# beer-asr/beer

Hardware: AMD Instinct MI355X
Metric: frames/sec per VB iteration (E+M) (higher is better)
Workload: dtype f32

## Files before the change

### beer_amd/csrc/estep_bf16.hip

```cpp

#include <cstdlib>
#include <type_traits>
#include <utility>

#include "estep_mfma.h"
#include "estep_tiles.h"

namespace beer_mfma {

namespace {

typedef __bf16 bf8 __attribute__((ext_vector_type(8)));
typedef unsigned int u4 __attribute__((ext_vector_type(4)));
typedef float f32x2 __attribute__((ext_vector_type(2)));

template <int V> using ic = std::integral_constant<int, V>;
template <int... I, typename F>
__device__ __forceinline__ void static_for_impl(std::integer_sequence<int, I...>, F&& f) {
    (f(ic<I>{}), ...);
}
template <int N, typename F>
__device__ __forceinline__ void static_for(F&& f) {
    static_for_impl(std::make_integer_sequence<int, N>{}, static_cast<F&&>(f));
}

constexpr int NP = kPackedPieces;
constexpr int kProdA[6] = {0, 0, 1, 0, 1, 2};
constexpr int kProdB[6] = {0, 1, 0, 2, 1, 0};

__device__ __forceinline__ bf8 as_bf8(const u4& w) { return __builtin_bit_cast(bf8, w); }
__device__ __forceinline__ f32x4 mfma_bf16(const u4& a, const u4& b, const f32x4& c) {
    return __builtin_amdgcn_mfma_f32_16x16x32_bf16(as_bf8(a), as_bf8(b), c, 0, 0, 0);
}
template <bool FIRST>
__device__ __forceinline__ void mfma_bf16_pinned(f32x4& acc, const u4& a, const u4& b) {
    if (FIRST)
        asm volatile("s_nop 1\n\tv_mfma_f32_16x16x32_bf16 %0, %1, %2, %0" : "+a"(acc) : "v"(a), "v"(b));
    else
        asm volatile("v_mfma_f32_16x16x32_bf16 %0, %1, %2, %0" : "+a"(acc) : "v"(a), "v"(b));
}
__device__ __forceinline__ void mfma_drain() {
    asm volatile("s_nop 15\n\ts_nop 15" ::: "memory");
    __builtin_amdgcn_sched_barrier(0);
}

__host__ __device__ inline size_t frame_image_tile_u4(int nk_used, int nqt) {
    return (size_t)(nk_used * NP * 2 + nqt * NP) * 64;
}
__host__ __device__ constexpr int img_nqt(int nk_used) { return nk_used <= 3 ? 5 : 6; }
constexpr int kImgMaxNK = 4;
__host__ __device__ inline int stat_slab(int j) { return j + j / 7; }
__host__ __device__ inline int nk16_of(int cov, int D) {
    return ((nslabx_of(cov, D) + 7) / 8 + 1) / 2 * 2;
}
__host__ __device__ inline int ld16_of(int D) {
    const int ld = 4 * d4_of(D) + 8;
    return (ld / 4) % 2 ? ld : ld + 4;
}
constexpr float kConstEps = 5.9604644775390625e-8f;
constexpr int kBlockU4 = NP * 64;

__device__ inline double entry_value(int cov, int D, int K, int k, int slab, int e,
                                     const float* __restrict__ row, bool* is_const) {
    const int D4 = d4_of(D), Dp = 4 * D4, nslab = nslabx_of(cov, D);
    *is_const = false;
    if (slab >= nslab) return 0.0;
    if (band_layout(cov, D)) {
        const int nb = band_nslab(D);
        if (slab == nslab - 1) {
            *is_const = true;
            return 0.0;
        }
        if (k >= K) return 0.0;
        if (slab >= nb) {
            const int b = 4 * (slab - nb) + e;
            return b < D ? (double)row[b] : 0.0;
        }
        int a, b;
        if (!band_pair(D, slab, e, &a, &b)) return 0.0;
        return b == a ? -0.5 * (double)row[D + a * D + a]
                      : -0.5 * ((double)row[D + a * D + b] + (double)row[D + b * D + a]);
    }
    const int t = slab_entry(cov, D, slab);
    const int a = t & 0xff, b = ((t >> 8) & 0xff) + e, sq = t >> 16;
    if (a == Dp && b - e == Dp) {
        *is_const = true;
        return 0.0;
    }
    if (k >= K) return 0.0;
    if (sq) return b < D ? -0.5 * (double)row[cov == BEER_ISO ? D : D + b] : 0.0;
    if (a < D) {
        if (b >= D || b < a) return 0.0;
        return b == a ? -0.5 * (double)row[D + a * D + a]
                      : -0.5 * ((double)row[D + a * D + b] + (double)row[D + b * D + a]);
    }
    return b < D ? (double)row[b] : 0.0;
}

__global__ __launch_bounds__(256) void const_max_kernel(int cov, int D, int K,
                                                        const float* __restrict__ E,
                                                        const float* __restrict__ logw,
                                                        float* __restrict__ c0) {
    __shared__ double red[8];
    const int Q = stats_dim(cov, D);
    double m = -1.0e300;
    for (int k = threadIdx.x; k < K; k += blockDim.x) {
        const double v = const_total(cov, D, E + (size_t)k * Q, logw ? (double)logw[k] : 0.0);
        if (v == v && v > m && v < 1.0e300) m = v;
    }
    m = block_max(m, red);
    if (threadIdx.x == 0) c0[0] = m > -1.0e300 ? (float)m : 0.f;
}

__global__ __launch_bounds__(256) void packx_kernel(int cov, int D, int K, int NT,
                                                    const float* __restrict__ E,
                                                    const float* __restrict__ logw,
                                                    unsigned short* __restrict__ P,
                                                    int* __restrict__ tab, int G, int Gp,
                                                    const float* __restrict__ c0, int lane_major) {
    extern __shared__ __attribute__((aligned(16))) char pack_lds[];
    const int nk = nk16_of(cov, D), nent = nk * 32;
    const int slot = blockIdx.x;
    const int k = slot % Gp < G ? (slot / Gp) * G + slot % Gp : K;
    const int chunk = slot / (NT * 16), kk = slot % (NT * 16);
    const int c = lane_major ? kk % NT : 4 * (kk / 64) + (kk % 4);
    const int i = lane_major ? kk / NT : (kk % 64) / 4;
    if (slot == 0)
        for (int s = threadIdx.x; s < (nk + 1) * 8; s += blockDim.x) tab[s] = slabx_entry(cov, D, s);
    const int Qs = stats_dim(cov, D);
    float* rowl = reinterpret_cast<float*>(pack_lds);
    if (k < K)
        for (int q = threadIdx.x; q < Qs; q += blockDim.x) rowl[q] = E[(size_t)k * Qs + q];
    __syncthreads();
    unsigned short* base = P + ((size_t)chunk * nk * NT) * (NP * 512);
    auto put = [&](int q, float v) {
        const int s = q / 32, g = (q % 32) / 8, j = q % 8;
        unsigned short* dst = base + ((size_t)s * NT + c) * (NP * 512) + (g * 16 + i) * 8 + j;
        unsigned short p[3];
        split3_scalar(v, p);
        dst[0] = p[0];
        dst[512] = p[1];
        dst[1024] = p[2];
    };
    const int nslab = nslabx_of(cov, D);
    for (int q = threadIdx.x; q < nent; q += blockDim.x) {
        bool is_const;
        const double v = entry_value(cov, D, K, k, q / 4, q % 4, rowl, &is_const);
        if (!is_const) {
            put(q, (float)v);
        } else if (q % 4 == 0) {
            const bool last = q / 4 == nslab - 1;
            const double want = k < K ? const_share(cov, D, q / 4, rowl, logw ? (double)logw[k] : 0.0) -
                                            (last ? (double)c0[0] : 0.0)
                                      : (last ? kPadLogit : 0.0);
            const float hi = (float)want;
            const double rem = (want - (double)hi) * (1.0 / (double)kConstEps);
            put(q, hi);
            put(q + 1, (rem == rem && fabs(rem) < 1.0e30) ? (float)rem : 0.f);
            put(q + 2, 0.f);
            put(q + 3, 0.f);
        }
    }
}

inline int xcd_chunk_group(int ny, size_t chunk_bytes) {
    int cg = (int)((size_t)(2 << 20) / (chunk_bytes ? chunk_bytes : 1));
    return cg < 1 ? 1 : (cg > ny ? ny : cg);
}
inline unsigned xcd_grid(int64_t nx, int ny, int cg) {
    return (unsigned)((nx + 7) / 8 * 8 * cg * ((ny + cg - 1) / cg));
}
__device__ inline bool xcd_block(int64_t nx, int ny, int cg, int64_t& bx, int& by) {
    const unsigned per_group = (unsigned)((nx + 7) / 8 * 8 * cg);
    const unsigned grp = blockIdx.x / per_group, rem = blockIdx.x - grp * per_group;
    const unsigned xcd = rem & 7, slot = rem >> 3;
    by = (int)(grp * cg + slot % (unsigned)cg);
    bx = (int64_t)(slot / (unsigned)cg) * 8 + xcd;
    return bx < nx && by < ny;
}

template <int FW>
__device__ __forceinline__ void stage_rows(const float* __restrict__ X, int64_t fb,
                                           int64_t nframes, int D, int LD, int lane,
                                           float* __restrict__ xw) {
    const int Dp = 4 * d4_of(D);
    if ((D & 3) == 0) {
        constexpr int LPR = 64 / FW, NPC = kMaxDimX / 4 / LPR;
        const int C4 = D >> 2, r = lane & (FW - 1), h = lane / FW;
        const int64_t f = fb + r;
        const bool valid = f < nframes;
        const f32x4* src = reinterpret_cast<const f32x4*>(X) + (valid ? f : nframes - 1) * C4;
        f32x4 xv[NPC];
#pragma unroll
        for (int it = 0; it < NPC; ++it) {
            const int pc = h + LPR * it;
            xv[it] = src[pc < C4 ? pc : C4 - 1];
        }
#pragma unroll
        for (int it = 0; it < NPC; ++it) {
            const int pc = h + LPR * it;
            if (pc < C4)
                *reinterpret_cast<f32x4*>(xw + r * LD + 4 * pc) =
                    valid ? xv[it] : f32x4{0.f, 0.f, 0.f, 0.f};
        }
        for (int idx = lane; idx < FW * ((LD - D) / 4); idx += 64) {
            const int rr = idx / ((LD - D) / 4), hh = idx - rr * ((LD - D) / 4);
            *reinterpret_cast<f32x4*>(xw + rr * LD + D + 4 * hh) =
                f32x4{hh == 0 ? 1.f : 0.f, hh == 0 ? kConstEps : 0.f, 0.f, 0.f};
        }
    } else {
        for (int idx = lane; idx < FW * LD; idx += 64) {
            const int r = idx / LD, c = idx - r * LD;
            const int64_t f = fb + r;
            float v = 0.f;
            if (c < D) { if (f < nframes) v = X[f * D + c]; }
            else if (c == Dp) v = 1.f;
            else if (c == Dp + 1) v = kConstEps;
            xw[idx] = v;
        }
    }
}

template <int NT, int MT, int GQ, bool PACKED, bool SQ, bool LNO, bool IMG = false, bool BL = false>
__global__ __launch_bounds__(kThreads, 2) void llhx_kernel(
    int64_t nframes, int D, int K, int S, int G, int gl, int jw, int nk,
    const float* __restrict__ X, const u4* __restrict__ Pall, const int* __restrict__ tab,
    float* __restrict__ resps, float* __restrict__ log_norm, double* __restrict__ llh_sum,
    float* __restrict__ xt_out, int xt_floats, int nku, int cg, const float* __restrict__ c0,
    const u4* __restrict__ img = nullptr) {
    static_assert(MT * NT <= 32, "128 accumulators: two waves per SIMD (launch bounds)");
    static_assert(!IMG || (MT == 2 && !PACKED && LNO), "the image holds 32-frame tiles");
    static_assert(!BL || (NT == 16 && MT == 2 && !IMG), "half k-steps of 8 tiles, hipcc-scheduled form");
    extern __shared__ __attribute__((aligned(16))) char smem[];
    const int LD = ld16_of(D);
    const int Dp = 4 * d4_of(D);
    const int tid = threadIdx.x, lane = tid & 63;
    const int wave = __builtin_amdgcn_readfirstlane(tid >> 6);
    const int i = lane & 15, g = lane >> 4;
    constexpr int FW = 16 * MT, NW = kThreads / 64;
    float* xw = reinterpret_cast<float*>(smem) + wave * (FW * LD);
    int* tabs = reinterpret_cast<int*>(reinterpret_cast<float*>(smem) + NW * FW * LD);
    constexpr int kHalfBytes = 8 * kBlockU4 * 16;
    char* ring = smem + (((size_t)NW * FW * LD * sizeof(float) + (size_t)(nk + 1) * 8 * sizeof(int)
                          + 1023) & ~(size_t)1023);
    int64_t bx = blockIdx.x;
    int by = 0;
    {
        const int nch = (K + 16 * NT - 1) / (16 * NT);
        constexpr int FBK = FW * NW;
        if (nch > 1 && !xcd_block((nframes + FBK - 1) / FBK, nch, cg, bx, by)) return;
    }
    const int64_t fb = (bx * NW + wave) * FW;
    for (int idx = tid; idx < (nk + 1) * 8; idx += kThreads) tabs[idx] = tab[idx];
    if (!IMG) stage_rows<FW>(X, fb, nframes, D, LD, lane, xw);
    __syncthreads();
    if (IMG && fb >= nframes) return;
    {
        static_assert(64 % FW == 0, "whole waves per 64-frame tile");
        if (xt_out && by == 0 && fb < (nframes + 63) / 64 * 64) {
            float* img = xt_out + (fb / 64) * (size_t)xt_floats;
            const int c0 = (int)(fb % 64);
            const int ncol4 = FW / 4 + (c0 + FW == 64 ? 1 : 0);
            for (int e4 = lane; e4 < (D + 2) * ncol4; e4 += 64) {
                const int row = e4 / ncol4, c = 4 * (e4 - row * ncol4);
                f32x4 v = {0.f, 0.f, 0.f, 0.f};
                if (row < D) {
#pragma unroll
                    for (int j = 0; j < 4; ++j) v[j] = c + j < FW ? xw[(c + j) * LD + row] : 0.f;
                } else if (row == D) {
                    v = f32x4{1.f, 1.f, 1.f, 1.f};
                }
                __builtin_nontemporal_store(v, reinterpret_cast<f32x4*>(img + row * 68 + c0 + c));
            }
        }
    }

    f32x4 acc[MT][NT];
#pragma unroll
    for (int m = 0; m < MT; ++m)
#pragma unroll
        for (int c = 0; c < NT; ++c) acc[m][c] = f32x4{0, 0, 0, 0};

    const float* xrow[MT];
#pragma unroll
    for (int m = 0; m < MT; ++m) xrow[m] = xw + (m * 16 + i) * LD;

    const int kbase = by * (16 * NT);
    const u4* Pl = Pall + (size_t)by * nk * NT * kBlockU4 + lane;
    const int* tl = tabs + 2 * g;

    struct AFrag { u4 w[NP][MT]; };
    auto make_half = [&](int s, int m, int h, AFrag& f) {
        const int t = tl[8 * s + h];
        f32x4 p;
        if constexpr (SQ) {
            const int a = t & 0xff, j = (t >> 8) & 0xff;
            const bool sq = (t >> 16) != 0;
            const f32x4 bb = *reinterpret_cast<const f32x4*>(xrow[m] + j);
            const float xx = xrow[m][a];
#pragma unroll
            for (int e = 0; e < 4; ++e) p[e] = bb[e] * (sq ? bb[e] : xx);
        } else {
            const f32x4 bb = *reinterpret_cast<const f32x4*>(xrow[m] + (t & 0xff));
#pragma unroll
            for (int e = 0; e < 4; ++e) p[e] = bb[e] * xrow[m][band_col(t, e, Dp)];
        }
#pragma unroll
        for (int e = 0; e < 2; ++e) {
            unsigned w3[3];
            split3(p[2 * e], p[2 * e + 1], w3);
#pragma unroll
            for (int q = 0; q < NP; ++q) f.w[q][m][2 * h + e] = w3[q];
        }
    };
    constexpr int BT = 2, NBATCH = NT / BT;
    static_assert(NT % BT == 0 && NBATCH % 2 == 0, "B batches alternate between two buffers");
    struct BFrag { u4 p[BT][NP]; };
    auto load_b = [&](int64_t blk, BFrag& b) {
#pragma unroll
        for (int c = 0; c < BT; ++c)
#pragma unroll
            for (int q = 0; q < NP; ++q) {
                if constexpr (BL) {
                    const int bb = (int)(blk + c);
                    b.p[c][q] = *reinterpret_cast<const u4*>(
                        ring + ((bb >> 3) & 1) * kHalfBytes + (bb & 7) * (kBlockU4 * 16) + q * 1024 +
                        lane * 16);
                } else {
                    b.p[c][q] = Pl[(size_t)(blk + c) * kBlockU4 + 64 * q];
                }
            }
    };
    typedef __attribute__((address_space(3))) void* lds_ptr;
    const char* bsrc = reinterpret_cast<const char*>(Pall + (size_t)by * nk * NT * kBlockU4) +
                       wave * 1024 + lane * 16;
    auto stage_half = [&](int hs) {
        const char* src = bsrc + (size_t)hs * kHalfBytes;
        char* dst = ring + (hs & 1) * kHalfBytes + wave * 1024;
#pragma unroll
        for (int n = 0; n < kHalfBytes / 1024 / NW; ++n)
            __builtin_amdgcn_global_load_lds(reinterpret_cast<const u4*>(src + n * (NW * 1024)),
                                             (lds_ptr)(dst + n * (NW * 1024)), 16, 0, 0);
    };
    auto publish = [&]() {
        asm volatile("s_waitcnt vmcnt(0) lgkmcnt(0)" ::: "memory");
        __builtin_amdgcn_s_barrier();
    };
    auto batch = [&](int s, int bi, const AFrag& cur, AFrag& nxt, const BFrag& b, BFrag& bn) {
        if constexpr (BL) {
            if (bi == NBATCH / 2 - 1 || bi == NBATCH - 1) {
                publish();
                const int hs = 2 * (s + 1) + (bi == NBATCH - 1 ? 1 : 0);
                if (hs < 2 * nku) stage_half(hs);
            }
        }
        load_b((int64_t)s * NT + (bi + 1) * BT, bn);
        if constexpr (!IMG) {
#pragma unroll
            for (int hh = bi * MT * 2 / NBATCH; hh < (bi + 1) * MT * 2 / NBATCH; ++hh)
                make_half(s + 1, hh % MT, hh / MT, nxt);
        }
#pragma unroll
        for (int pr = 0; pr < 6; ++pr)
#pragma unroll
            for (int c = 0; c < BT; ++c)
#pragma unroll
                for (int m = 0; m < MT; ++m)
                    acc[m][bi * BT + c] = mfma_bf16(cur.w[kProdA[pr]][m], b.p[c][kProdB[pr]],
                                                    acc[m][bi * BT + c]);
        if constexpr (BL)
            __builtin_amdgcn_sched_group_barrier(0x100, NP * BT, 0);
        else
            __builtin_amdgcn_sched_group_barrier(0x020, NP * BT, 0);
        if constexpr (!IMG)
            __builtin_amdgcn_sched_group_barrier(0x100, 2 * ((MT * 2 + NBATCH - 1) / NBATCH), 0);
        __builtin_amdgcn_sched_group_barrier(0x008, 6 * MT * BT, 0);
    };
    const u4* ti = nullptr;
    if constexpr (IMG)
        ti = img + (fb / FW) * (int64_t)frame_image_tile_u4(nku, img_nqt(nku)) + lane;
    auto load_a = [&](int s, AFrag& f) {
#pragma unroll
        for (int q = 0; q < NP; ++q)
#pragma unroll
            for (int m = 0; m < MT; ++m) f.w[q][m] = ti[((s * NP + q) * MT + m) * 64];
    };
    auto kstep = [&](int s, const AFrag& cur, AFrag& nxt, BFrag& b0, BFrag& b1) {
        if constexpr (IMG) {
            if (s + 1 < nku) load_a(s + 1, nxt);
        }
#pragma unroll
        for (int bi = 0; bi < NBATCH; bi += 2) {
            batch(s, bi, cur, nxt, b0, b1);
            batch(s, bi + 1, cur, nxt, b1, b0);
        }
    };
    AFrag f0, f1;
    BFrag b0, b1;
    if constexpr (IMG) {
        load_a(0, f0);
    } else {
#pragma unroll
        for (int hh = 0; hh < MT * 2; ++hh) make_half(0, hh % MT, hh / MT, f0);
    }
    if constexpr (BL) {
        stage_half(0);
        if (nku > 0) stage_half(1);
        publish();
    }
    load_b(0, b0);
    for (int s = 0; s < nku; s += 2) {
        kstep(s, f0, f1, b0, b1);
        if (s + 1 < nku) kstep(s + 1, f1, f0, b0, b1);
    }
    if constexpr (LNO) {
        if constexpr (NT == 16 && GQ == 1) {
            if (gl == 0) {
                if (G == 4)
                    lognorm_epilogue_lane_major<NT, MT, 4>(acc, fb, nframes, kbase, S, i, g, lane, log_norm, llh_sum, c0[0]);
                else if (G == 8)
                    lognorm_epilogue_lane_major<NT, MT, 8>(acc, fb, nframes, kbase, S, i, g, lane, log_norm, llh_sum, c0[0]);
                else
                    lognorm_epilogue_lane_major<NT, MT, 16>(acc, fb, nframes, kbase, S, i, g, lane, log_norm, llh_sum, c0[0]);
                return;
            }
        }
#define BEER_LN(GL_) lognorm_epilogue<NT, MT, GQ, GL_>(acc, fb, nframes, kbase, S, G, i, g, lane, \
                                                       log_norm, llh_sum, c0[0])
        switch (gl) {
            case 1: BEER_LN(1); break;
            case 2: BEER_LN(2); break;
            case 4: BEER_LN(4); break;
            case 8: BEER_LN(8); break;
            default: BEER_LN(16); break;
        }
#undef BEER_LN
    } else {
        softmax_epilogue<float, NT, MT, GQ, PACKED, LNO>(acc, fb, nframes, kbase, K, S, G, gl, jw,
                                                         i, g, lane, resps, log_norm, llh_sum,
                                                         c0[0]);
    }
}

inline bool k1_lds_fits(int D, int nk) {
    size_t lds = (size_t)32 * (kThreads / 64) * ld16_of(D) * sizeof(float) + (size_t)(nk + 1) * 8 * sizeof(int);
    lds = ((lds + 1023) & ~(size_t)1023) + 2 * (size_t)(8 * kBlockU4 * 16);
    return 2 * lds <= (size_t)beer::kMaxDynLds;
}

thread_local int g_cov_of_launch = BEER_FULL;

template <int NT, int MT, int GQ, bool PACKED = false, bool SQ = true, bool LNO = false,
          bool IMG = false, bool BL = false>
int launch_llhx(int64_t nframes, int D, int K, int S, int G, int gl, int jw, int nchunks, int nk,
                const float* X, const void* P, const int* tab, const float* c0, float* resps,
                float* log_norm, double* llh_sum, hipStream_t s, float* xt_out = nullptr,
                int xt_floats = 0, const void* img = nullptr) {
    const int LD = ld16_of(D);
    const int nku = (nslabx_of(SQ ? g_cov_of_launch : BEER_FULL, D) + 7) / 8;
    constexpr int FB = 16 * MT * (kThreads / 64);
    size_t lds = (size_t)FB * LD * sizeof(float) + (size_t)(nk + 1) * 8 * sizeof(int);
    if (BL) lds = ((lds + 1023) & ~(size_t)1023) + 2 * (size_t)(8 * kBlockU4 * 16);
    const int64_t blocks = (nframes + FB - 1) / FB;
    if (nchunks != (K + 16 * NT - 1) / (16 * NT)) return BEER_EINVAL;
    const int cg = xcd_chunk_group(nchunks, (size_t)nku * NT * kBlockU4 * 16);
    (void)hipFuncSetAttribute(
        reinterpret_cast<const void*>(llhx_kernel<NT, MT, GQ, PACKED, SQ, LNO, IMG, BL>),
        hipFuncAttributeMaxDynamicSharedMemorySize, beer::kMaxDynLds);
    hipLaunchKernelGGL((llhx_kernel<NT, MT, GQ, PACKED, SQ, LNO, IMG, BL>),
                       dim3(nchunks > 1 ? xcd_grid(blocks, nchunks, cg) : (unsigned)blocks),
                       dim3(kThreads), lds, s, nframes, D, K, S, G, gl, jw, nk, X,
                       reinterpret_cast<const u4*>(P), tab, resps, log_norm, llh_sum, xt_out,
                       xt_floats, nku, cg, c0, reinterpret_cast<const u4*>(img));
    BEER_LAUNCH_CHECK();
    return BEER_OK;
}

constexpr int kAxFT = 64;
constexpr int kAxXS = kAxFT + 4;
constexpr int kPiece = 4096;
constexpr int kAxMC = 8, kAxWaves = 4;

inline int xt_rows(int D) { return D + 2; }
inline int xt_pieces(int D) { return (xt_rows(D) * kAxXS * 4 + kPiece - 1) / kPiece; }

__global__ __launch_bounds__(256) void xt_image_kernel(int64_t nframes, int D, int NX,
                                                       const float* __restrict__ X,
                                                       float* __restrict__ Xt) {
    constexpr int LD = kMaxDimX + 1;
    __shared__ float tile[kAxFT * LD];
    const int64_t tau = blockIdx.x, t0 = tau * kAxFT;
    const int rows = (int)(nframes - t0 < kAxFT ? nframes - t0 : kAxFT);
    for (int e = threadIdx.x; e < rows * D; e += 256) {
        const int f = e / D, d = e - f * D;
        tile[f * LD + d] = X[t0 * D + e];
    }
    __syncthreads();
    float* out = Xt + tau * ((size_t)NX * (kPiece / 4));
    for (int e = threadIdx.x; e < NX * (kPiece / 4); e += 256) {
        const int row = e / kAxXS, col = e - row * kAxXS;
        float v = 0.f;
        if (row < D) v = col < rows ? tile[col * LD + row] : 0.f;
        else if (row == D) v = 1.f;
        __builtin_nontemporal_store(v, out + e);
    }
}

template <bool SR, int NQ>
__global__ __launch_bounds__(64 * kAxWaves, 1) void accx_kernel(
    int64_t nframes, int D, int K, int nslab, int NX, const float* __restrict__ Xt,
    const unsigned* __restrict__ Rimg, const int* __restrict__ tab,
    int64_t frames_per_block, double* __restrict__ Sp, int gx, int gy, int gz,
    const float* __restrict__ Gt, int lgG, int sx, int band) {
    constexpr int MC = kAxMC, WAVES = kAxWaves, NB = 2;
    static_assert(16 * MC == kPackedComps && kAxFT == kPackedFrames, "the packed image is this kernel's LDS tile");
    constexpr int plane = kPackedPlaneWords * 4;
    const int r_off = NX * kPiece, buf_bytes = r_off + NP * plane;
    const int xstride = sx ? 0 : buf_bytes;
    const int rstride = sx ? NP * plane : buf_bytes;
    const int g_base = sx ? r_off + NB * NP * plane : NB * buf_bytes;
    extern __shared__ __attribute__((aligned(16))) char smem[];
    const int tid = threadIdx.x, lane = tid & 63;
    const int wave = __builtin_amdgcn_readfirstlane(tid >> 6);
    const int i = lane & 15, g = lane >> 4;
    const int D4 = d4_of(D), Dp = 4 * D4, nq = nslab * 4;
    const int id = blockIdx.x, xcd = id & 7, slot0 = id >> 3;
    const int bx = slot0 % gx;
    const int yz = (slot0 / gx) * 8 + xcd;
    if (yz >= gy * gz) return;
    const int by = yz % gy, bz = yz / gy;
    const int tile0 = (bx * WAVES + wave) * NQ;
    const int kc0 = by * (16 * MC);
    const int64_t tb = (int64_t)bz * frames_per_block;
    const int64_t te = tb + frames_per_block < nframes ? tb + frames_per_block : nframes;
    const int ntiles = (int)((te - tb + kAxFT - 1) / kAxFT);
    const int64_t tau0 = tb / kAxFT;
    const int nblk = (K + 16 * MC - 1) / (16 * MC);
    const int gbytes = SR ? ((16 * MC) >> lgG) * kAxFT * 4 : 0;
    const int gkb = (gbytes + 1023) >> 10;

    auto factors = [&](int uu, int& a, int& b) {
        const int col = 16 * (tile0 + uu) + i, slab = col >> 2;
        a = b = Dp + 2;
        if (slab < nslab) {
            const int t = tab[slab];
            if (band) {
                a = (t & 0xff) + (col & 3);
                b = band_col(t, col & 3, Dp);
            } else {
                b = ((t >> 8) & 0xff) + (col & 3);
                a = (t >> 16) ? b : (t & 0xff);
            }
        }
    };
    int xa_off[NQ], xb_off[NQ];
#pragma unroll
    for (int uu = 0; uu < NQ; ++uu) {
        int a, b;
        factors(uu, a, b);
        xa_off[uu] = ((a < D ? a : (a == Dp ? D : D + 1)) * kAxXS + 8 * g) * 4;
        xb_off[uu] = ((b < D ? b : (b == Dp ? D : D + 1)) * kAxXS + 8 * g) * 4;
    }
    int a_off[kAxFT / 32];
#pragma unroll
    for (int ks = 0; ks < kAxFT / 32; ++ks)
        a_off[ks] = r_off + (i * kPackedFrames + (((4 * ks + g) ^ (i & 7)) << 3)) * 2;

    f32x4 acc[MC][NQ];
#pragma unroll
    for (int c = 0; c < MC; ++c)
#pragma unroll
        for (int uu = 0; uu < NQ; ++uu) acc[c][uu] = f32x4{0, 0, 0, 0};

    static_assert((kPiece / 1024) % WAVES == 0 && (NP * plane / 1024) % WAVES == 0,
                  "regions are whole rounds of the waves");
    const char* xsrc = reinterpret_cast<const char*>(Xt) + wave * 1024 + lane * 16;
    const char* rsrc = reinterpret_cast<const char*>(Rimg) + wave * 1024 + lane * 16;
    const char* gsrc = SR ? reinterpret_cast<const char*>(Gt) + wave * 1024 + lane * 16 : nullptr;
    typedef __attribute__((address_space(3))) void* lds_ptr;
    auto stage_x = [&](int tile, int buf) {
        const char* xs = xsrc + (tau0 + tile) * (size_t)(NX * kPiece);
        char* dst = smem + buf * xstride + wave * 1024;
#pragma unroll 1
        for (int n = 0; n < NX * (kPiece / 1024) / WAVES; ++n)
            __builtin_amdgcn_global_load_lds(reinterpret_cast<const u4*>(xs + n * (WAVES * 1024)),
                                             (lds_ptr)(dst + n * (WAVES * 1024)), 16, 0, 0);
    };
    auto stage_r = [&](int tile, int buf) {
        const int64_t tau = tau0 + tile;
        const char* rs = rsrc + (tau * nblk + by) * (size_t)(NP * plane);
        char* dst = smem + r_off + buf * rstride + wave * 1024;
#pragma unroll
        for (int n = 0; n < NP * plane / 1024 / WAVES; ++n)
            __builtin_amdgcn_global_load_lds(reinterpret_cast<const u4*>(rs + n * (WAVES * 1024)),
                                             (lds_ptr)(dst + n * (WAVES * 1024)), 16, 0, 0);
        if (SR && wave < gkb)
            __builtin_amdgcn_global_load_lds(
                reinterpret_cast<const u4*>(gsrc + (tau * nblk + by) * (size_t)gbytes),
                (lds_ptr)(smem + g_base + buf * 4096 + wave * 1024), 16, 0, 0);
    };
    auto stage = [&](int tile, int buf) {
        if (!sx) stage_x(tile, buf);
        stage_r(tile, buf);
    };
    auto fold = [&](int buf) {
#pragma unroll 1
        for (int n = 0; n < 16 * MC * 8 / (64 * WAVES); ++n) {
            const int p = tid + 64 * WAVES * n, c = p >> 3, pos = p & 7, ch = pos ^ (c & 7);
            char* ph = smem + buf * rstride + r_off + c * (kPackedFrames * 2) + pos * 16;
            const u4 w0 = *reinterpret_cast<const u4*>(ph);
            const u4 w1 = *reinterpret_cast<const u4*>(ph + plane);
            const u4 w2 = *reinterpret_cast<const u4*>(ph + 2 * plane);
            const float* gm = reinterpret_cast<const float*>(smem + g_base + buf * 4096) +
                              ((c >> lgG) * kAxFT + 8 * ch);
            const f32x4 g0 = *reinterpret_cast<const f32x4*>(gm);
            const f32x4 g1 = *reinterpret_cast<const f32x4*>(gm + 4);
            u4 o0, o1, o2;
#pragma unroll
            for (int wd = 0; wd < 4; ++wd) {
                const float lo = (__builtin_bit_cast(float, w1[wd] << 16) +
                                  __builtin_bit_cast(float, w2[wd] << 16)) +
                                 __builtin_bit_cast(float, w0[wd] << 16);
                const float hi = (__builtin_bit_cast(float, w1[wd] & 0xffff0000u) +
                                  __builtin_bit_cast(float, w2[wd] & 0xffff0000u)) +
                                 __builtin_bit_cast(float, w0[wd] & 0xffff0000u);
                const float ga = wd < 2 ? g0[2 * wd] : g1[2 * wd - 4];
                const float gb = wd < 2 ? g0[2 * wd + 1] : g1[2 * wd - 3];
                unsigned w3[3];
                split3(lo * ga, hi * gb, w3);
                o0[wd] = w3[0]; o1[wd] = w3[1]; o2[wd] = w3[2];
            }
            *reinterpret_cast<u4*>(ph) = o0;
            *reinterpret_cast<u4*>(ph + plane) = o1;
            *reinterpret_cast<u4*>(ph + 2 * plane) = o2;
        }
    };
    if (ntiles > 0) {
        stage_x(0, 0);
        stage_r(0, 0);
    }
    __syncthreads();
    if (SR && ntiles > 0) {
        fold(0);
        __syncthreads();
    }
    const bool active = tile0 * 16 < nq;
    u4 af[MC][NP], bf[2][NP];
    constexpr int kPA[6] = {0, 0, 0, 1, 1, 2}, kPB[6] = {0, 1, 2, 0, 1, 0};
    auto a_ptr = [&](int b, int ks, int c) {
        return smem + a_off[ks] + (b * rstride + c * 16 * kPackedFrames * 2);
    };
    auto load_a = [&](int b, int ks) {
#pragma unroll
        for (int q = 0; q < NP; ++q)
#pragma unroll
            for (int c = 0; c < MC; ++c)
                af[c][q] = *reinterpret_cast<const u4*>(a_ptr(b, ks, c) + q * plane);
    };
    auto gen_b = [&](int b, int ks, int uu, u4 (&out)[NP]) {
        const char* pa = smem + xa_off[uu] + (b * xstride + 128 * ks);
        const char* pb = smem + xb_off[uu] + (b * xstride + 128 * ks);
        const f32x4 xa0 = *reinterpret_cast<const f32x4*>(pa);
        const f32x4 xa1 = *reinterpret_cast<const f32x4*>(pa + 16);
        const f32x4 xb0 = *reinterpret_cast<const f32x4*>(pb);
        const f32x4 xb1 = *reinterpret_cast<const f32x4*>(pb + 16);
        const f32x4 p0 = xa0 * xb0, p1 = xa1 * xb1;
#pragma unroll
        for (int e = 0; e < 4; ++e) {
            unsigned w3[3];
            split3(e < 2 ? p0[2 * e] : p1[2 * e - 4], e < 2 ? p0[2 * e + 1] : p1[2 * e - 3], w3);
#pragma unroll
            for (int q = 0; q < NP; ++q) out[q][e] = w3[q];
        }
    };
    if (active && ntiles > 0) gen_b(0, 0, 0, bf[0]);
    auto iteration = [&](int tile, int buf) __attribute__((always_inline)) {
        const int next = buf ^ 1;
        if (tile + 1 < ntiles) stage(tile + 1, next);
        const bool fold_next = SR && tile + 1 < ntiles;
        if (active) {
#pragma unroll
            for (int ks = 0; ks < 2; ++ks) {
                load_a(buf, ks);
#pragma unroll
                for (int uu = 0; uu < NQ; ++uu) {
                    const int cur = (ks * NQ + uu) & 1;
                    const bool build = uu + 1 < NQ || ks == 0;
                    const int nks = uu + 1 < NQ ? ks : 1, nuu = uu + 1 < NQ ? uu + 1 : 0;
                    const char* pa = smem + xa_off[nuu] + (buf * xstride + 128 * nks);
                    const char* pb = smem + xb_off[nuu] + (buf * xstride + 128 * nks);
                    f32x4 xa[2], xb[2];
                    float pp[8];
                    Split3Steps st[4];
#pragma unroll
                    for (int n = 0; n < 6 * MC; ++n) {
                        const int pr = n / MC, c = n % MC;
                        mfma_bf16_pinned<false>(acc[c][uu], af[c][kPA[pr]], bf[cur][kPB[pr]]);
                        if (!build) continue;
                        if (n == 1) xa[0] = *reinterpret_cast<const f32x4*>(pa);
                        else if (n == 2) xa[1] = *reinterpret_cast<const f32x4*>(pa + 16);
                        else if (n == 3) xb[0] = *reinterpret_cast<const f32x4*>(pb);
                        else if (n == 4) xb[1] = *reinterpret_cast<const f32x4*>(pb + 16);
                        else if (n >= 12 && n < 20) {
                            const int e = n - 12;
                            asm volatile("v_mul_f32 %0, %1, %2" : "=v"(pp[e])
                                         : "v"(xa[e >> 2][e & 3]), "v"(xb[e >> 2][e & 3]));
                        } else if (n >= 20) {
                            constexpr int NCH = 2;
                            const int m = n - 20, grp = m / (7 * NCH), mm = m % (7 * NCH);
                            const int e = NCH * grp + mm % NCH;
                            split3_step(mm / NCH, pp[2 * e], pp[2 * e + 1], st[e]);
                        }
                    }
                    if (build) {
#pragma unroll
                        for (int e = 0; e < 4; ++e) {
                            bf[cur ^ 1][0][e] = st[e].w0;
                            bf[cur ^ 1][1][e] = st[e].w1;
                            bf[cur ^ 1][2][e] = st[e].w2;
                        }
                    }
                }
            }
        }
        __syncthreads();
        if (sx && tile + 1 < ntiles) {
            stage_x(tile + 1, 0);
            __syncthreads();
        }
        if (SR) {
            if (fold_next) fold(next);
            __syncthreads();
        }
        if (active && tile + 1 < ntiles) gen_b(next, 0, 0, bf[0]);
    };
    for (int tile = 0; tile < ntiles; tile += NB) {
        iteration(tile, 0);
        if (tile + 1 < ntiles) iteration(tile + 1, 1);
    }
    mfma_drain();
#pragma unroll
    for (int uu = 0; uu < NQ; ++uu) {
        const int q = (tile0 + uu) * 16 + i;
        if (q >= nq) continue;
#pragma unroll
        for (int c = 0; c < MC; ++c)
#pragma unroll
// ... 1392 lines not shown
```

Baseline: 247.0 million.

## Hand-interleave A-fragment generation and B loads with pinned MFMAs in BL path

For the band-layout (BL) kernel variant, each batch becomes a hand-scheduled stream. Pinned inline-asm MFMAs are interleaved with LDS loads of the next B fragments, address computation, raw X loads and split3 steps for the next A fragment. The table words are pre-packed into 6-bit column indices so addresses come from bitfield extracts rather than band_col evaluation. This hides the fragment-building latency behind MFMA issue, but it relies on manual hazard handling (s_nop, drain) and is restricted to leading dimensions of 64 or less and non-SQ configurations.

```diff
diff --git a/beer_amd/csrc/estep_bf16.hip b/beer_amd/csrc/estep_bf16.hip
--- a/beer_amd/csrc/estep_bf16.hip
+++ b/beer_amd/csrc/estep_bf16.hip
@@ -38,6 +38,9 @@
         asm volatile("s_nop 1\n\tv_mfma_f32_16x16x32_bf16 %0, %1, %2, %0" : "+a"(acc) : "v"(a), "v"(b));
     else
         asm volatile("v_mfma_f32_16x16x32_bf16 %0, %1, %2, %0" : "+a"(acc) : "v"(a), "v"(b));
+}
+__device__ __forceinline__ void mfma_bf16_pinned_v(f32x4& acc, const u4& a, const u4& b) {
+    asm volatile("v_mfma_f32_16x16x32_bf16 %0, %1, %2, %0" : "+v"(acc) : "v"(a), "v"(b));
 }
 __device__ __forceinline__ void mfma_drain() {
     asm volatile("s_nop 15\n\ts_nop 15" ::: "memory");
@@ -221,6 +224,13 @@
     }
 }
 
+__device__ __forceinline__ int k1_slab_word(int t, int Dp) {
+    int w = t & 0xff;
+#pragma unroll
+    for (int e = 0; e < 4; ++e) w |= band_col(t, e, Dp) << (6 + 6 * e);
+    return w;
+}
+
 template <int NT, int MT, int GQ, bool PACKED, bool SQ, bool LNO, bool IMG = false, bool BL = false>
 __global__ __launch_bounds__(kThreads, 2) void llhx_kernel(
     int64_t nframes, int D, int K, int S, int G, int gl, int jw, int nk,
@@ -230,7 +240,7 @@
     const u4* __restrict__ img = nullptr) {
     static_assert(MT * NT <= 32, "128 accumulators: two waves per SIMD (launch bounds)");
     static_assert(!IMG || (MT == 2 && !PACKED && LNO), "the image holds 32-frame tiles");
-    static_assert(!BL || (NT == 16 && MT == 2 && !IMG), "half k-steps of 8 tiles, hipcc-scheduled form");
+    static_assert(!BL || (NT == 16 && MT == 2 && !IMG && !SQ), "half k-steps of 8 tiles, band slabs");
     extern __shared__ __attribute__((aligned(16))) char smem[];
     const int LD = ld16_of(D);
     const int Dp = 4 * d4_of(D);
@@ -251,7 +261,8 @@
         if (nch > 1 && !xcd_block((nframes + FBK - 1) / FBK, nch, cg, bx, by)) return;
     }
     const int64_t fb = (bx * NW + wave) * FW;
-    for (int idx = tid; idx < (nk + 1) * 8; idx += kThreads) tabs[idx] = tab[idx];
+    for (int idx = tid; idx < (nk + 1) * 8; idx += kThreads)
+        tabs[idx] = BL ? k1_slab_word(tab[idx], Dp) : tab[idx];
     if (!IMG) stage_rows<FW>(X, fb, nframes, D, LD, lane, xw);
     __syncthreads();
     if (IMG && fb >= nframes) return;
@@ -301,9 +312,10 @@
 #pragma unroll
             for (int e = 0; e < 4; ++e) p[e] = bb[e] * (sq ? bb[e] : xx);
         } else {
-            const f32x4 bb = *reinterpret_cast<const f32x4*>(xrow[m] + (t & 0xff));
-#pragma unroll
-            for (int e = 0; e < 4; ++e) p[e] = bb[e] * xrow[m][band_col(t, e, Dp)];
+            const f32x4 bb = *reinterpret_cast<const f32x4*>(xrow[m] + (t & (BL ? 0x3f : 0xff)));
+#pragma unroll
+            for (int e = 0; e < 4; ++e)
+                p[e] = bb[e] * xrow[m][BL ? (t >> (6 + 6 * e)) & 0x3f : band_col(t, e, Dp)];
         }
 #pragma unroll
         for (int e = 0; e < 2; ++e) {
@@ -346,13 +358,80 @@
         asm volatile("s_waitcnt vmcnt(0) lgkmcnt(0)" ::: "memory");
         __builtin_amdgcn_s_barrier();
     };
+    static_assert(!BL || 4 * MT == NBATCH, "one unit of fragment arithmetic per batch");
+    struct ARaw { f32x4 bb; float xc[4]; };
+    typedef __attribute__((address_space(3))) const float* lds_cf;
+    typedef __attribute__((address_space(3))) const f32x4* lds_cf4;
+    ARaw raw[2];
+    int th[2];
+    unsigned ad[5], rowb[MT];
+#pragma unroll
+    for (int m = 0; m < MT; ++m) rowb[m] = (unsigned)(size_t)(lds_cf)xrow[m];
+    auto addr_step = [&](int k, int m, int h) {
+#define BEER_AD(K_, LO_)                                                                     \
+    case K_:                                                                                 \
+        asm volatile("v_bfe_u32 %0, %1, " #LO_ ", 6\n\tv_lshl_add_u32 %0, %0, 2, %2"         \
+                     : "=&v"(ad[K_]) : "v"(th[h]), "v"(rowb[m]));                            \
+        break;
+        switch (k) {
+            BEER_AD(0, 0) BEER_AD(1, 6) BEER_AD(2, 12) BEER_AD(3, 18) BEER_AD(4, 24)
+            default: break;
+        }
+#undef BEER_AD
+    };
+    auto load_raw = [&](int k, ARaw& r) {
+        if (k == 0) r.bb = *(lds_cf4)ad[0];
+        else r.xc[k - 1] = *(lds_cf)ad[k];
+    };
+    auto batch_stream = [&](int s, int bi, const AFrag& cur, AFrag& nxt, const BFrag& b, BFrag& bn) {
+        if (bi == NBATCH / 2 - 1 || bi == NBATCH - 1) {
+            publish();
+            const int hs = 2 * (s + 1) + (bi == NBATCH - 1 ? 1 : 0);
+            if (hs < 2 * nku) stage_half(hs);
+        }
+        const int bb0 = s * NT + (bi + 1) * BT;
+        const int hu = bi / 2, mu = hu % MT, wu = 2 * (hu / MT) + bi % 2, eu = bi % 2;
+        const ARaw& ru = raw[hu & 1];
+        const int hl = (bi / 2 + 1) % (MT * 2);
+        float pp[2];
+        Split3Steps st;
+#pragma unroll
+        for (int n = 0; n < 6 * MT * BT; ++n) {
+            const int pr = n / (MT * BT), c = n / MT % BT, m = n % MT, k = n / 2;
+            mfma_bf16_pinned_v(acc[m][bi * BT + c], cur.w[kProdA[pr]][m], b.p[c][kProdB[pr]]);
+            if (n % 2 == 0) {
+                const int kb = bi % 2 ? k - 5 : k - 1;
+                if (kb >= 0 && kb < NP * BT) {
+                    const int blk = bb0 + kb % BT;
+                    bn.p[kb % BT][kb / BT] = *reinterpret_cast<const u4*>(
+                        ring + ((blk >> 3) & 1) * kHalfBytes + (blk & 7) * (kBlockU4 * 16) +
+                        (kb / BT) * 1024 + lane * 16);
+                } else if (bi % 2) {
+                    if (k < 5) load_raw(k, raw[hl & 1]);
+                } else if (k >= 7) {
+                    addr_step(k - 7, hl % MT, hl / MT);
+                } else if (bi == NBATCH / 2 - 2) {
+                    th[1] = tl[8 * (s + 1) + 1];
+                } else if (bi == NBATCH - 2) {
+                    th[0] = tl[8 * min(s + 2, nk)];
+                }
+            } else if (k == 0) {
+                asm volatile("v_mul_f32 %0, %2, %3\n\tv_mul_f32 %1, %4, %5"
+                             : "=&v"(pp[0]), "=&v"(pp[1])
+                             : "v"(ru.bb[2 * eu]), "v"(ru.xc[2 * eu]), "v"(ru.bb[2 * eu + 1]),
+                               "v"(ru.xc[2 * eu + 1]));
+            } else if (k < 8) {
+                split3_step(k - 1, pp[0], pp[1], st);
+            }
+        }
+        nxt.w[0][mu][wu] = st.w0;
+        nxt.w[1][mu][wu] = st.w1;
+        nxt.w[2][mu][wu] = st.w2;
+    };
     auto batch = [&](int s, int bi, const AFrag& cur, AFrag& nxt, const BFrag& b, BFrag& bn) {
         if constexpr (BL) {
-            if (bi == NBATCH / 2 - 1 || bi == NBATCH - 1) {
-                publish();
-                const int hs = 2 * (s + 1) + (bi == NBATCH - 1 ? 1 : 0);
-                if (hs < 2 * nku) stage_half(hs);
-            }
+            batch_stream(s, bi, cur, nxt, b, bn);
+            return;
         }
         load_b((int64_t)s * NT + (bi + 1) * BT, bn);
         if constexpr (!IMG) {
@@ -368,10 +447,7 @@
                 for (int m = 0; m < MT; ++m)
                     acc[m][bi * BT + c] = mfma_bf16(cur.w[kProdA[pr]][m], b.p[c][kProdB[pr]],
                                                     acc[m][bi * BT + c]);
-        if constexpr (BL)
-            __builtin_amdgcn_sched_group_barrier(0x100, NP * BT, 0);
-        else
-            __builtin_amdgcn_sched_group_barrier(0x020, NP * BT, 0);
+        __builtin_amdgcn_sched_group_barrier(0x020, NP * BT, 0);
         if constexpr (!IMG)
             __builtin_amdgcn_sched_group_barrier(0x100, 2 * ((MT * 2 + NBATCH - 1) / NBATCH), 0);
         __builtin_amdgcn_sched_group_barrier(0x008, 6 * MT * BT, 0);
@@ -409,10 +485,21 @@
         publish();
     }
     load_b(0, b0);
+    if constexpr (BL) {
+        th[0] = tl[8];
+#pragma unroll
+        for (int k = 0; k < 5; ++k) {
+            addr_step(k, 0, 0);
+            load_raw(k, raw[0]);
+        }
+        __builtin_amdgcn_sched_barrier(0);
+        asm volatile("s_nop 1");
+    }
     for (int s = 0; s < nku; s += 2) {
         kstep(s, f0, f1, b0, b1);
         if (s + 1 < nku) kstep(s + 1, f1, f0, b0, b1);
     }
+    if constexpr (BL) mfma_drain();
     if constexpr (LNO) {
         if constexpr (NT == 16 && GQ == 1) {
             if (gl == 0) {
@@ -443,6 +530,7 @@
 }
 
 inline bool k1_lds_fits(int D, int nk) {
+    if (ld16_of(D) > 64) return false;
     size_t lds = (size_t)32 * (kThreads / 64) * ld16_of(D) * sizeof(float) + (size_t)(nk + 1) * 8 * sizeof(int);
     lds = ((lds + 1023) & ~(size_t)1023) + 2 * (size_t)(8 * kBlockU4 * 16);
     return 2 * lds <= (size_t)beer::kMaxDynLds;
```

Result: faster. 257.2 million (median of 6 runs) (+4.1%).
